# thalesfm/differentiable-renderer

Measured on AMD Instinct MI355X. Metric: Mray/s (fwd+bwd), Cornell 512x512 @64spp depth 8, higher is better.
Workload: dtype f32; 1 GPU; config 3: Cornell 512x512, 64 spp, depth 8, fwd + radiative backprop w.r.t. the albedos; scene 'cornell' (cornell box of render.cpp:26-59) 512x512, 64 spp per GPU, depth 8 (-b 8 -p 1), fwd + radiative-backprop gradients of 4 parameters; program=builtin, parallelism=1 GPU, gpu_max_hw_queues=4 (set by this script before the HIP runtime started)

## Files before the change

differentiable-renderer_amd/csrc/drt_ctx.h:

```cpp
#pragma once

namespace {

struct DevBuf {
    void* p = nullptr;
    size_t cap = 0;
};

struct TimedLaunch {
    int kernel;
    hipEvent_t e0, e1;
};

struct NormalEqRequest {
    const float* d_target = nullptr;
    const float* d_residual = nullptr;
    float* d_jacobian = nullptr;
    double *d_A = nullptr, *d_b = nullptr, *d_loss = nullptr;
    bool cross = false;
    double* d_bias = nullptr;
    float* d_variance = nullptr;
};
struct ParamSetsRequest {
    int n_sets = 0, width = 0;
// ... 33 lines not shown
    float* out_gimg = nullptr;
    drt_hip_stats* stats = nullptr;
    int gimg_param = -1;
    bool tangent = false;
    bool second_image() const { return gimg_param >= 0 || tangent; }
    bool backward = false, dev_out = false, timing = false, want_segments = false, sync = true;
    bool zero_copy = false;
    bool direct_out = false, direct_gimg = false;
    uint64_t done_seq = 0;
    bool copy_kernel = false;
    int n_shards = 1, shard = 0, band = 1;
    uint32_t n_local_pixels = 0;
    size_t n_count_words = 0;
    float* d_out = nullptr;
    float* d_gimg = nullptr;
    size_t off_grad = 0, off_img = 0, off_gimg = 0, off_adj = 0, img_bytes = 0, grad_bytes = 0;
    drt_hip_stats st;
    std::chrono::steady_clock::time_point t0;
};

}

struct drt_hip_ctx {
    int device = 0;
    int n_cu = 256;
    uint64_t device_mem = (uint64_t)288 << 30;
    int mesh_blocks_per_cu = 4;
    hipStream_t stream = nullptr;
    std::string err;

    bool has_scene = false;
    bool has_specular = false;
    bool emissive_bxdf = false;
    int max_colour_param = -1;
    unsigned colour_mask = 0, emission_mask = 0;
    bool prog_ok = false;
    bool prog_sorted = false;
    unsigned long long prog_sig[4] = {0, 0, 0, 0};
    std::string arch = "gfx950";
    int jit_mode = 1;
    uint64_t scene_work = 0;
    std::map<std::string, hipFunction_t> jit_fn;
    std::vector<hipModule_t> jit_modules;
    std::string user_header;
    std::string jit_error;
    double jit_ms = 0;
    int n_params = 0, n_shapes = 0;
    int n_user_params = 0;
    int n_grad_slots = 0;
    std::vector<uint8_t> requires_grad;
    std::vector<drt_material_desc> materials;
    DevScene<float>* d_scene_f = nullptr;
    DevScene<double>* d_scene_d = nullptr;
    float* d_params_f = nullptr;
    double* d_params_d = nullptr;
    bool has_mesh = false;
    DevBvh<float> bvh_f{};
    DevBvh<double> bvh_d{};
    std::vector<void*> mesh_allocs;

    hipStream_t path_stream[2] = {nullptr, nullptr};
    hipEvent_t ev_begin[2] = {nullptr, nullptr}, ev_path[2] = {nullptr, nullptr};
    hipEvent_t ev_lane_free[2] = {nullptr, nullptr};
    bool lane_used[2] = {false, false};
    hipEvent_t ev_params = nullptr;
    bool params_pending[2] = {false, false};
// ... 114 lines not shown
```

differentiable-renderer_amd/csrc/drt_path.h:

```cpp
#pragma once

#include "drt_kernels.h"

#define DRT_DRAW_TABLE (3 * DRT_MAX_DEPTH + 8)

struct PathArgs {
    int32_t W, H, spp;
    int32_t shard, n_shards, band;
    uint32_t Pb, p0, Sb, s0, spr, n_ranges, n_groups;
    int32_t min_bounces, depth_cap, cap_is_roulette, cap_draws;
    uint32_t rr_threshold, seed, rng_stream;
    uint32_t regen_min;
    uint32_t shade_min, descend_min;
    int32_t gimg_param;
    uint32_t gen_rows, gen_clog2;
    uint32_t hist_lds, hist_stride;
    uint32_t gimg_row, pad_gen;
    unsigned long long hist_ovf;
    double p_rr, inv_p_rr;
    double eye[3], fwd[3], right[3], up[3];
    double tan_half, aspect, inv_W, inv_H;
    float p_rr_f, inv_p_rr_f;
    float eye_f[3], fwd_f[3], right_f[3], up_f[3], cs_step_f, ct_step_f;
    __host__ __device__ uint32_t dirs_out() const { return gen_rows; }
// ... 4 lines not shown
{
    uint32_t ly = lp / (uint32_t)a.W, x = lp - ly * (uint32_t)a.W;
    uint32_t y = ly;
    if (a.n_shards > 1) {
        uint32_t b = ly / (uint32_t)a.band, r = ly - b * (uint32_t)a.band;
        y = (b * (uint32_t)a.n_shards + (uint32_t)a.shard) * (uint32_t)a.band + r;
    }
    return y * (uint32_t)a.W + x;
}

template <typename SG>
__device__ inline HitRec<float> path_closest_hit(const DevScene<float>* __restrict__ sc, const ProgRecs<SG::n>& recs, float4 ra, float2 rb)
{
    return closest_hit_prog<SG>(sc, recs, mk<float>(ra.x, ra.y, ra.z), mk<float>(ra.w, rb.x, rb.y));
}
template <typename SG>
__device__ inline HitRec<double> path_closest_hit(const DevScene<double>* __restrict__ sc, const ProgRecs<SG::n, double>& recs, double4 ra, double2 rb)
{
    if (SG::n > 0)
        return closest_hit_sig<SG, double>(recs, mk<double>(ra.x, ra.y, ra.z), mk<double>(ra.w, rb.x, rb.y));
    const double4 ra1[1] = {ra};
    const double2 rb1[1] = {rb};
    HitRec<double> h1[1];
    closest_hit_n<double, 1>(sc, sc->n_shapes, ra1, rb1, h1);
    return h1[0];
}

#define DRT_SIG_CORNELL                                                                                                   \
    ((unsigned long long)DRT_PK_SPHERE | (unsigned long long)DRT_PK_SPHERE << 3 | (unsigned long long)DRT_PK_AX << 6 |    \
     (unsigned long long)DRT_PK_PLANE << 9 | (unsigned long long)DRT_PK_AZ << 12 | (unsigned long long)DRT_PK_AZ << 15 |  \
     (unsigned long long)DRT_PK_AY << 18 | (unsigned long long)DRT_PK_AY << 21 | (unsigned long long)DRT_PK_SPHERE << 24)
#define DRT_NSIG_CORNELL 9
typedef KindSig<DRT_SIG_CORNELL, 0ull, 0ull, 0ull, DRT_NSIG_CORNELL> SigCornell;


template <typename R>
struct PathSceneLds {
    struct {
        int n_shapes, n_materials, n_emitters, n_params;
        DevShape<R> shapes[DRT_MAX_SHAPES];
        DevMaterial<R> materials[DRT_MAX_MATERIALS];
        int emitter_param[DRT_MAX_EMITTERS];
        int flat[DRT_MAX_SHAPES];
    } sc;
    R params[DRT_PATH_LDS_PARAMS * 3];
#ifdef DRT_USER_SHAPES
    R user_q[DRT_MAX_SHAPES][4];
#endif
};

template <typename R, bool ALL_LDS = false>
__device__ inline V3<R> load_param(const PathSceneLds<R>& lds, const R* __restrict__ params, int id)
{
    if (ALL_LDS || id < DRT_PATH_LDS_PARAMS)
        return mk<R>(lds.params[id * 3], lds.params[id * 3 + 1], lds.params[id * 3 + 2]);
    return mk<R>(params[id * 3], params[id * 3 + 1], params[id * 3 + 2]);
}
template <typename R>
struct SetParams {
    const R* p;
};
template <typename R, bool ALL_LDS = false>
__device__ inline V3<R> load_param(const SetParams<R>& set, const R* __restrict__, int id)
{
    return mk<R>(set.p[id * 3], set.p[id * 3 + 1], set.p[id * 3 + 2]);
}
// ... 107 lines not shown
#ifndef DRT_LEAN_PATH_MIN_BLOCKS
#define DRT_LEAN_PATH_MIN_BLOCKS 8
#endif
#ifndef DRT_REGEN_MIN_BLOCKS
#define DRT_REGEN_MIN_BLOCKS 5
#endif
#ifndef DRT_F64_MIN_BLOCKS
#define DRT_F64_MIN_BLOCKS 4
#endif
#ifndef DRT_TANGENT_MIN_BLOCKS
#define DRT_TANGENT_MIN_BLOCKS 6
#endif
#ifndef DRT_TANGENT_REGEN_MIN_BLOCKS
#define DRT_TANGENT_REGEN_MIN_BLOCKS 5
#endif
#ifndef DRT_TANGENT_F64_MIN_BLOCKS
#define DRT_TANGENT_F64_MIN_BLOCKS 3
#endif
#ifndef DRT_TANGENTS2_MIN_BLOCKS
#define DRT_TANGENTS2_MIN_BLOCKS 5
#endif
#ifndef DRT_TANGENTS4_MIN_BLOCKS
#define DRT_TANGENTS4_MIN_BLOCKS 3
#endif
#ifndef DRT_TANGENTS8_MIN_BLOCKS
#define DRT_TANGENTS8_MIN_BLOCKS 2
#endif
#ifndef DRT_GEN_TABLE
#define DRT_GEN_TABLE 408
#endif
template <bool B, typename X, typename Y> struct PickT { typedef X T; };
template <typename X, typename Y> struct PickT<false, X, Y> { typedef Y T; };
struct NoLds { int unused; };
template <typename R> struct GenAcc { typedef double T; };
#ifdef DRT_GEN_F32
template <> struct GenAcc<float> { typedef float T; };
#endif

template <typename R>
struct GenLds {
    R colnz[DRT_PATH_LDS_PARAMS][4];
    R invc[DRT_PATH_LDS_PARAMS][4];
    static __device__ inline const GenLds* over_invc(const R* rows) { return reinterpret_cast<const GenLds*>(rows - DRT_PATH_LDS_PARAMS * 4); }
};

template <typename R, typename SL>
__device__ inline void stage_gen(GenLds<R>& gl, const SL& lds, const DevScene<R>* __restrict__ sc)
{
    for (int p = threadIdx.x; p < DRT_PATH_LDS_PARAMS; p += blockDim.x) {
        const bool in = p < lds.sc.n_params;
        uint32_t zinc = 0, zbits = 0;
#pragma unroll
        for (int ch = 0; ch < 3; ++ch) {
            const R c = in ? lds.params[p * 3 + ch] : R(1);
            const bool zero = zero_channel(c);
            gl.colnz[p][ch] = zero ? R(1) : c;
            gl.invc[p][ch] = zero ? R(0) : R(1) / c;
            zinc |= zero ? 1u << (8 * ch) : 0u;
            zbits |= zero ? 1u << ch : 0u;
        }
        const uint32_t slot = in ? (uint32_t)sc->grad_slot[p] : DRT_SLOT_NONE;
        gl.colnz[p][3] = pid_pack(R(0), zinc);
        gl.invc[p][3] = pid_pack(R(0), slot | zbits << 16);
    }
    __syncthreads();
}
// ... 552 lines not shown
                    a0 = ap;
                if (is_colour) {
                    const uint32_t n = (tg.cnt[p >> 2] >> (8 * (p & 3))) & 0xFFu;
                    const R nf = (R)(int)n;
                    V3<R> dT = mk<R>(Tr.x * (nf * tl.invc[p][0]), Tr.y * (nf * tl.invc[p][1]), Tr.z * (nf * tl.invc[p][2]));
                    const uint32_t zb = __builtin_amdgcn_readfirstlane(tl.inc[p][3]);
                    if (zb) {
                        const bool one = n == 1u;
                        if (zb & 1u) dT.x = (one && (tg.zc & 0xFFu) == 0x1u) ? T.x : R(0);
                        if (zb & 2u) dT.y = (one && (tg.zc & 0xFF00u) == 0x100u) ? T.y : R(0);
                        if (zb & 4u) dT.z = (one && (tg.zc & 0xFF0000u) == 0x10000u) ? T.z : R(0);
                    }
                    tg.acc_set(p, mk<R>(fma_r(dT.x, gE.x, a0.x), fma_r(dT.y, gE.y, a0.y), fma_r(dT.z, gE.z, a0.z)));
                } else
                    tg.acc_set(p, a0);
            }
        }
    }
}

template <typename R>
struct CameraLane {
    R cs0, ct0;
};

template <typename R>
struct PathVertex {
    V3<R> P, nrm, d;
    uint32_t ids;
    int material;
    bool hit, scattered;
};

template <typename R, bool SPEC, int NP, int NC, typename SG, bool FREEZE_BY_ROW = false, bool FIXED = false, bool NO_LIT_BXDF = false>
__device__ inline void path_bounce(const PathArgs& a, const PathSceneLds<R>& lds, const TangentLds<R>& tl, const DevScene<R>* __restrict__ sc,
                                   const R* __restrict__ params, const ProgRecs<SG::n, R>& recs, uint32_t key,
                                   R pk, R inv_pk, uint32_t n_theta, bool next_rr, bool next_cap, bool live, V3<R> g,
                                   typename Q4<R>::T& ra, typename Q2<R>::T& rb, V3<R>& T, V3<R>& L, Tangents<R, NP, NC>& tg,
                                   bool& alive, bool& capped, bool& on_light, uint32_t& light, PathVertex<R>* vo = nullptr,
                                   bool last = false, const float* __restrict__ seed_px = nullptr, const uint32_t* ih = nullptr)
{
    auto draw = [&](uint32_t n) { return ih ? drt_rng_combine(ih[n], key) : rng_draw(a.rng_stream, key, n); };
    const HitRec<R> h = path_closest_hit<SG>(sc, recs, ra, rb);
    const bool hit = live && h.prim >= 0;
    const int prim = h.prim >= 0 ? h.prim : 0;
    const V3<R> o = mk<R>(ra.x, ra.y, ra.z);
    const V3<R> d = mk<R>(ra.w, rb.x, rb.y);
    const V3<R> P = o + d * h.t;
    const DevShape<R>& sh = lds.sc.shapes[prim];
    const uint32_t ids = (uint32_t)sh.pad;
    const uint32_t cid = ids & 0xFFFFu, eid = ids >> 16;
    const bool has_bxdf = cid != DRT_ID_NONE, emits = hit && eid != DRT_ID_NONE;
    on_light = emits && !has_bxdf;
    light = eid;
    if (last && !vo) {
        if constexpr (!NO_LIT_BXDF) if (wave_any(emits && has_bxdf)) {
            if (emits && has_bxdf) {
                if (NP != 0 && seed_px)
                    g = mk<R>((R)seed_px[0], (R)seed_px[1], (R)seed_px[2]);
                add_emission<R, NP, NC>(lds, tl, params, eid, inv_pk, T, g, L, tg);
            }
        }
        alive = false;
        capped = false;
        if constexpr (!FIXED) if (!a.cap_is_roulette) {
            const bool rr_kills = next_rr && draw(n_theta + 2) < a.rr_threshold;
            capped = hit && has_bxdf && !rr_kills;
        }
        return;
    }
    const V3<R> ctr = mk<R>(sh.p[0], sh.p[1], sh.p[2]);
    const V3<R> nsph = normalize(P - ctr);
    const bool is_plane = sh.type == DRT_SHAPE_PLANE;
    V3<R> nrm = mk<R>(is_plane ? ctr.x : nsph.x, is_plane ? ctr.y : nsph.y, is_plane ? ctr.z : nsph.z);
#ifdef DRT_USER_SHAPES
// ... 549 lines not shown
            counts[(size_t)a.n_groups * a.n_ranges + w] = n_capped;
        }
    }
    if constexpr (GEN || SGRAD)
        gen_finish(s_gen, a, gpart);
    else
    if constexpr (NP > 0 && !JAC) {
        const int wv = threadIdx.x / DRT_WAVE;
        double (*red)[DRT_FAST_PARAMS * 3] = s_red;
        if (REGEN) {
            __syncthreads();
            red = reinterpret_cast<double (*)[DRT_FAST_PARAMS * 3]>(&s_film[0][0]);
        }
#pragma unroll
        for (int r = 0; r < NP * 3; ++r) {
            double v = (double)tg.acc[r * DRT_BLOCK];
#pragma unroll
            for (int o2 = DRT_WAVE / 2; o2 > 0; o2 >>= 1)
                v += __shfl_down(v, o2);
            if (lane == 0)
                red[wv][r] = v;
        }
        __syncthreads();
        if (threadIdx.x < DRT_FAST_PARAMS * 3) {
            double v = 0;
            if ((int)threadIdx.x < NP * 3)
                for (int ww = 0; ww < DRT_BLOCK / DRT_WAVE; ++ww)
                    v += red[ww][threadIdx.x];
            gpart[(size_t)blockIdx.x * (DRT_FAST_PARAMS * 3) + threadIdx.x] = v;
        }
    }
}

template <typename R, int NP, int NCR, typename SG>
__global__ void __launch_bounds__(DRT_BLOCK, (SG::n <= DRT_LEAN_MAX_SHAPES ? DRT_LEAN_PATH_MIN_BLOCKS : DRT_LOCKSTEP_GEN_MIN_BLOCKS))
k_path_lean(PathArgs a, const DevScene<R>* __restrict__ sc, const R* __restrict__ params, const float* __restrict__ adjoint,
            double* __restrict__ gpart, double* __restrict__ fpart, uint32_t* __restrict__ counts,
            unsigned long long* __restrict__ total, double* __restrict__ gimg_part)
{
    static_assert(sizeof(R) == 4 && (NP == 0 || NP == 4), "k_path_lean: f32, four parameters in columns or none");
    static_assert(!DRT_JACOBIAN_OF(NCR), "k_path_lean has no Jacobian form");
    (void)gimg_part;
    if (total && blockIdx.x == 0 && threadIdx.x < 8)
        total[threadIdx.x] = 0;
    typedef typename Q4<R>::T R4;
    typedef typename Q2<R>::T R2;
    constexpr int NC = DRT_NC_OF(NCR), ROLES = DRT_ROLES_OF(NCR);
    __shared__ PathSceneLds<R> lds;
    __shared__ double s_red[DRT_BLOCK / DRT_WAVE][DRT_FAST_PARAMS * 3];
    __shared__ TangentLds<R> s_tl;
    stage_path_scene(lds, sc, params);
    const TangentLds<R>& tl = s_tl;
    if (NC > 0)
        stage_tangents(s_tl, lds);

    const uint32_t lane = threadIdx.x & (DRT_WAVE - 1);
    const uint32_t w = grid_wave();
    const uint32_t range = w / a.n_groups, group = w - range * a.n_groups;
    const uint32_t lp = group * DRT_WAVE + lane;
    const bool have = range < a.n_ranges && lp < a.Pb;
    const uint32_t s_begin = range * a.spr;
    const uint32_t s_end = s_begin + a.spr < a.Sb ? s_begin + a.spr : a.Sb;

    Tangents<R, NP, NC> tg;
    __shared__ R s_acc[NP > 0 ? NP * 3 : 1][DRT_BLOCK];
    tg.acc = &s_acc[0][threadIdx.x];
#pragma unroll
    for (int p = 0; p < NP; ++p)
        tg.acc_set(p, mk<R>(R(0), R(0), R(0)));
    double fx = 0, fy = 0, fz = 0;
    uint32_t n_seg = 0;

    uint32_t gpix = 0, px = 0, py = 0;
    V3<R> g = mk<R>(R(1), R(1), R(1));
// ... 4 lines not shown
        if (NP != 0 && adjoint)
            g = mk<R>((R)adjoint[(size_t)gpix * 3], (R)adjoint[(size_t)gpix * 3 + 1], (R)adjoint[(size_t)gpix * 3 + 2]);
    }
    CameraLane<R> cl;
    cl.cs0 = (R)((2. * (double)px * a.inv_W - 1.) * a.aspect * a.tan_half);
    cl.ct0 = (R)((2. * (double)py * a.inv_H - 1.) * a.tan_half);
    constexpr bool ARGS_F32 = DRT_CAMERA_ARGS_F32 != 0 && SG::n <= DRT_LEAN_MAX_SHAPES;
    ProgRecs<SG::n, R> recs;
    __shared__ typename PickT<(SG::n == 0), ProgLds, NoLds>::T s_prog;
    recs.lds = reinterpret_cast<const ProgLds*>(&s_prog);
    if (SG::n > 0)
        recs.template load<SG>(sc);
    if constexpr (SG::n == 0) {
        const DevScene<float>* scf = reinterpret_cast<const DevScene<float>*>(sc);
        if (threadIdx.x < DRT_PROG_SORTED_MAX) {
            s_prog.rec[threadIdx.x] = *reinterpret_cast<const float4*>(scf->sorted[threadIdx.x]);
            s_prog.shape[threadIdx.x] = scf->sorted_shape[threadIdx.x];
        }
        if (threadIdx.x < 8)
            s_prog.kind_begin[threadIdx.x] = scf->kind_begin[threadIdx.x];
        __syncthreads();
    }

    if (range < a.n_ranges) {
        for (uint32_t sl = s_begin; sl < s_end; ++sl) {
            R4 ra;
            R2 rb;
            const uint32_t key = path_camera<R, ARGS_F32>(a, cl, gpix, px, py, sl, ra, rb);
            bool live = have;
            V3<R> T = mk<R>(R(1), R(1), R(1)), L = mk<R>(R(0), R(0), R(0));
            uint32_t end_ids = DRT_ID_NONE;
            if (NC > 0)
                tg.new_path();
            for (int kk = 0; kk < a.depth_cap; ++kk) {
                const uint32_t n_live = (uint32_t)__popcll(wave_ballot(live));
                if (n_live == 0)
                    break;
                n_seg += n_live;
                const uint32_t n_theta = 2u * (uint32_t)kk + 2u;
                const bool next_cap = (kk + 1) >= a.depth_cap;
                bool alive, capped, on_light;
                uint32_t light;
                path_bounce<R, false, NP, NC, SG, (DRT_FREEZE_BY_ROW != 0 && SG::n <= DRT_LEAN_MAX_SHAPES), true, true>(
                    a, lds, tl, sc, params, recs, key, R(1), R(1), n_theta, false, next_cap, live, g, ra, rb, T, L, tg, alive, capped, on_light, light, nullptr, next_cap);
                end_ids = on_light ? light : end_ids;
                live = alive;
            }
            if (wave_any(end_ids != DRT_ID_NONE)) {
                if (end_ids != DRT_ID_NONE)
                    add_emission<R, NP, NC, false, PathSceneLds<R>, ROLES>(lds, tl, params, end_ids, R(1), T, g, L, tg);
            }
            fx += (double)L.x; fy += (double)L.y; fz += (double)L.z;
        }
        if (fpart && have) {
            double* f = fpart + ((size_t)range * 3) * a.Pb + lp;
            f[0] = fx; f[(size_t)a.Pb] = fy; f[(size_t)a.Pb * 2] = fz;
        }
        if (lane == 0) {
            counts[w] = n_seg;
            counts[(size_t)a.n_groups * a.n_ranges + w] = 0;
        }
    }
    if constexpr (NP > 0) {
        const int wv = threadIdx.x / DRT_WAVE;
#pragma unroll
        for (int r = 0; r < NP * 3; ++r) {
            double v = (double)tg.acc[r * DRT_BLOCK];
#pragma unroll
            for (int o2 = DRT_WAVE / 2; o2 > 0; o2 >>= 1)
                v += __shfl_down(v, o2);
            if (lane == 0)
                s_red[wv][r] = v;
        }
        __syncthreads();
        if (threadIdx.x < DRT_FAST_PARAMS * 3) {
            double v = 0;
// ... 706 lines not shown
```

differentiable-renderer_amd/csrc/drt_prog.h:

```cpp
#pragma once

#include "drt_device.h"

__device__ inline float prog_rcp(float x) { return __builtin_amdgcn_rcpf(x); }
__device__ inline double prog_rcp(double x) { return div_r(1.0, x); }
__device__ inline float prog_sqrt(float x) { return __builtin_amdgcn_sqrtf(x); }
__device__ inline double prog_sqrt(double x) { return sqrt_r(x); }

#ifdef DRT_USER_SHAPES
#include "drt_user_shapes.h"
template <int K, typename R>
__device__ inline bool user_intersect(const R* p, V3<R> o, V3<R> d, R& t)
{
    if (K == 0) return drt_user_intersect_0<R>(p, o, d, t);
    return drt_user_intersect_1<R>(p, o, d, t);
}
template <typename R>
__device__ inline V3<R> user_normal(int kind, const R* p, V3<R> P)
{
    if (kind == 0) return drt_user_normal_0<R>(p, P);
    return drt_user_normal_1<R>(p, P);
}
template <typename R>
__device__ inline void user_bxdf(int kind, const R* p, V3<R> n, V3<R> d, R u1, R u2, V3<R>& wo, R& pdf, R& bs)
// ... 111 lines not shown
};

template <typename SG, typename R>
__device__ inline HitRec<R> closest_hit_sig(const ProgRecs<SG::n, R>& recs, V3<R> o, V3<R> d)
{
    const V3<R> inv_d = mk<R>(prog_rcp(d.x), prog_rcp(d.y), prog_rcp(d.z));
    R tmin = (R)INFINITY;
    int prim = -1;
#pragma unroll
    for (int s = 0; s < SG::n; ++s) {
        const int kind = SG::kind(s);
        const typename Q4<R>::T r = recs.r[s];
        if (kind == DRT_PK_AX) prog_test<DRT_PK_AX, R>(r, s, o, d, inv_d, tmin, prim);
        else if (kind == DRT_PK_AY) prog_test<DRT_PK_AY, R>(r, s, o, d, inv_d, tmin, prim);
        else if (kind == DRT_PK_AZ) prog_test<DRT_PK_AZ, R>(r, s, o, d, inv_d, tmin, prim);
        else if (kind == DRT_PK_PLANE) prog_test<DRT_PK_PLANE, R>(r, s, o, d, inv_d, tmin, prim);
#ifdef DRT_USER_SHAPES
        else if (kind >= DRT_PK_USER0 && kind < DRT_PK_USER0 + DRT_MAX_USER_KINDS) {
            const typename Q4<R>::T q = recs.q[s];
            const R p8[8] = {r.x, r.y, r.z, r.w, q.x, q.y, q.z, q.w};
            R t;
            if (kind == DRT_PK_USER0 ? user_intersect<0, R>(p8, o, d, t) : user_intersect<1, R>(p8, o, d, t))
                prog_accept(t, s, tmin, prim);
        }
#endif
        else prog_test<DRT_PK_SPHERE, R>(r, s, o, d, inv_d, tmin, prim);
    }
    HitRec<R> h;
    h.t = tmin;
    h.prim = prim;
    return h;
}

template <typename SG>
__device__ inline HitRec<float> closest_hit_prog(const DevScene<float>* __restrict__ sc, const ProgRecs<SG::n>& recs,
                                                 V3<float> o, V3<float> d)
{
    (void)sc;
    if (SG::n > 0)
        return closest_hit_sig<SG, float>(recs, o, d);
    const V3<float> inv_d = mk<float>(__builtin_amdgcn_rcpf(d.x), __builtin_amdgcn_rcpf(d.y), __builtin_amdgcn_rcpf(d.z));
    float tmin = INFINITY;
    int prim = -1;
    {
        const ProgLds& pl = *recs.lds;
        bool tie = false;
#define DRT_KIND_LOOP(K)                                                              \
        for (int i = pl.kind_begin[K]; i < pl.kind_begin[K + 1]; ++i) {               \
            const float4 r = pl.rec[i];                                               \
            prog_test_tie<K>(r, pl.shape[i], o, d, inv_d, tmin, prim, tie);           \
        }
        DRT_KIND_LOOP(DRT_PK_AX)
        DRT_KIND_LOOP(DRT_PK_AY)
        DRT_KIND_LOOP(DRT_PK_AZ)
        DRT_KIND_LOOP(DRT_PK_PLANE)
        DRT_KIND_LOOP(DRT_PK_SPHERE)
#undef DRT_KIND_LOOP
        if (__any(tie && prim >= 0)) {
#define DRT_KIND_LOOP(K)                                                              \
            for (int i = pl.kind_begin[K]; i < pl.kind_begin[K + 1]; ++i) {           \
                const float4 r = pl.rec[i];                                           \
                prog_resolve_tie<K>(r, pl.shape[i], o, d, inv_d, tmin, prim);         \
            }
            DRT_KIND_LOOP(DRT_PK_AX)
            DRT_KIND_LOOP(DRT_PK_AY)
            DRT_KIND_LOOP(DRT_PK_AZ)
// ... 12 lines not shown
```

differentiable-renderer_amd/csrc/drt_render_impl.h:

```cpp
#pragma once

namespace {

int timing_begin(drt_hip_ctx* ctx, bool on, int kernel)
{
    if (!on)
        return DRT_OK;
    while (ctx->event_pool.size() < ctx->events_used + 2) {
        hipEvent_t e;
        HIPCHK(ctx, hipEventCreate(&e));
        ctx->event_pool.push_back(e);
    }
    TimedLaunch t;
    t.kernel = kernel;
    t.e0 = ctx->event_pool[ctx->events_used++];
    t.e1 = ctx->event_pool[ctx->events_used++];
    HIPCHK(ctx, hipEventRecord(t.e0, ctx->stream));
    ctx->timed.push_back(t);
    return DRT_OK;
}

int timing_end(drt_hip_ctx* ctx, bool on)
{
    if (!on)
// ... 84 lines not shown
        (S).st->launches[K]++;                                                     \
    } while (0)

template <int V>
using IntC = std::integral_constant<int, V>;
template <typename F>
auto with_bool(bool b, F&& f)
{
    return b ? f(std::true_type()) : f(std::false_type());
}
template <int V, int... Vs, typename F>
auto with_int(int v, F&& f)
{
    if constexpr (sizeof...(Vs) == 0)
        return v == V ? f(IntC<V>()) : decltype(f(IntC<V>()))();
    else
        return v == V ? f(IntC<V>()) : with_int<Vs...>(v, f);
}
inline int np_width(int n_params, int general)
{
    return n_params <= 4 ? 4 : (n_params <= 8 ? 8 : general);
}

enum class PathOp { biased, unbiased, mesh, tangent, jacobian, tangents, param_sets, param_sets_along, param_sets_grad, cross };
enum class PathProg { cornell, sorted, scene };
struct PathForm {
    PathOp op;
    bool f64, spec;
    int np, nc;
    bool regen;
    bool loss;
    int roles;
    bool fixed, no_lit_bxdf;
    PathProg prog;
    bool lean() const { return fixed && no_lit_bxdf; }
};

template <typename R>
struct Shard {
    typedef typename Q4<R>::T R4;
    typedef typename Q2<R>::T R2;
    drt_hip_ctx* ctx;
    const drt_camera_desc* cam;
    const drt_render_params* rp;
    const float* d_adjoint;
    float* d_out_rgb;
    bool backward, timing;
    drt_hip_stats* st;
    uint32_t n_local_pixels;
    int D;
    double* film;
    int gimg_param;
    double* gfilm;
    float* d_out_gimg;
    bool fwd_tangent;
    bool keep_sums;
    const NormalEqRequest* neq = nullptr;
    uint32_t neq_blocks = 0;
    int neq_vw = 1;
    int n_dirs = 0;
    const ParamSetsRequest* sets = nullptr;
    bool cross() const { return neq && neq->cross; }
    int jac_rows() const { return cross() ? n_dirs * 6 + 3 : (neq || sets) ? (n_dirs > 0 ? n_dirs : ctx->n_params) * (sets && sets->along ? 6 : 3) : 3; }
    bool sets_grad() const { return sets && sets->grad; }
    bool pixel_sums() const { return gimg_param >= 0 || fwd_tangent || neq || (sets && !sets->grad); }
    const DevScene<R>* d_scene;
// ... 48 lines not shown
    double *grad, *gpart;
    unsigned long long* totals;
    bool path_finished = false;

    int bounces_from(int k) const
    {
        if (!can_fuse)
            return 1;
        const int left = D - k;
        const int forced = tuning().shade_bounces > 0 ? tuning().shade_bounces : (rp->bounces_per_launch > 8 ? 8 : rp->bounces_per_launch);
        if (forced > 0)
            return forced < left ? forced : left;
        double alive = 1.0;
        int n = 0;
        while (n < left && n < 8) {
            alive *= 0.93 * ((k + n + 1) >= rp->min_bounces && (k + n + 1) < D ? 1.0 - rp->absorb : 1.0);
            ++n;
            if (alive < 0.1)
                break;
        }
        return n;
    }
};

inline std::string path_kernel_name(const drt_hip_ctx* ctx, const PathForm& f)
{
    const std::string sg = drt_jit::sig_type(ctx->prog_sig, ctx->n_shapes);
    const char* type = f.f64 ? "double" : "float";
    const char* sp = f.spec ? "true" : "false";
    char name[400];
    if (f.op == PathOp::unbiased)
        snprintf(name, sizeof name, "k_path_unbiased<%s, %s, %d, %s>", type, sp, f.np, sg.c_str());
    else if (f.lean())
        snprintf(name, sizeof name, "k_path_lean<%s, %d, %d, %s>", type, f.np, DRT_NC_ROLES(f.nc, 0, 0) | f.roles << 8, sg.c_str());
    else
        snprintf(name, sizeof name, "k_path<%s, %s, %d, %d, %s, %s%s>", type, sp, f.np,
                 DRT_NC_ROLES(f.nc, 0, 0) | f.roles << 8 | (f.op == PathOp::jacobian ? DRT_NC_JACOBIAN : 0), sg.c_str(), f.regen ? "true" : "false", f.loss ? ", true" : "");
    return name;
}

template <typename R>
unsigned path_dynamic_lds(const PathForm& f, int n_params, unsigned hist_bytes)
{
    const uint32_t n = (uint32_t)std::min(n_params, DRT_PATH_LDS_PARAMS), K = (uint32_t)f.nc;
    if (f.op == PathOp::tangents || f.op == PathOp::cross) return dirs_table_words(n, K) * (unsigned)sizeof(R);
    if (f.op == PathOp::param_sets) return sets_table_words(n, K) * (unsigned)sizeof(R);
    if (f.op == PathOp::param_sets_along) return sets_along_table_words(n, K) * (unsigned)sizeof(R);
    if (f.op == PathOp::param_sets_grad) return hist_bytes + sets_grad_table_words(n, K) * (unsigned)sizeof(R);
    return f.op == PathOp::unbiased ? 0u : hist_bytes;
}

template <typename R>
const void* library_path_kernel(const PathForm& f)
{
    if (f.loss || f.prog == PathProg::scene)
        return nullptr;
    const auto columns = [&f](auto k) {
        if (f.np == DRT_NP_ANY && f.nc == 0) return k(IntC<DRT_NP_ANY>(), IntC<0>());
        if (f.np == 8 && f.nc == 8) return k(IntC<8>(), IntC<8>());
        if (f.np == 4 && f.nc == 3) return k(IntC<4>(), IntC<3>());
        if (f.np == 4 && f.nc == 4) return k(IntC<4>(), IntC<4>());
        if (f.np == 0 && f.nc == 0) return k(IntC<0>(), IntC<0>());
        return (const void*)nullptr;
    };
    if (f.lean()) {
        if constexpr (sizeof(R) == 4) {
            if (f.np == 4 && f.nc == 3 && f.roles == DRT_ROLES_CORNELL)
                return with_bool(f.prog == PathProg::cornell, [](auto cornell) {
                    return (const void*)k_path_lean<R, 4, DRT_NC_ROLES(3, 0, 0) | DRT_ROLES_CORNELL << 8, std::conditional_t<cornell, SigCornell, SigNone>>; });
            if (f.np == 0 && f.nc == 0 && f.roles == 0)
                return with_bool(f.prog == PathProg::cornell, [](auto cornell) {
                    return (const void*)k_path_lean<R, 0, 0, std::conditional_t<cornell, SigCornell, SigNone>>; });
        }
        return nullptr;
    }
    const auto spec_sig = [&f](auto k) {
        return with_bool(f.spec, [&](auto spec) { return with_bool(f.prog == PathProg::cornell, [&](auto cornell) {
            return k(spec, std::conditional_t<cornell, SigCornell, SigNone>()); }); });
    };
    if (f.op == PathOp::jacobian) {
        if (f.regen || f.roles != 0)
            return nullptr;
        const auto jcols = [&f](auto k) {
            if (f.np == 8 && f.nc == 8) return k(IntC<8>(), IntC<8>());
            if (f.np == 4 && f.nc == 3) return k(IntC<4>(), IntC<3>());
            if (f.np == 4 && f.nc == 4) return k(IntC<4>(), IntC<4>());
            return (const void*)nullptr;
        };
        return jcols([&](auto np, auto nc) {
            return spec_sig([](auto spec, auto sg) {
                return (const void*)k_path<R, decltype(spec)::value, decltype(np)::value, decltype(nc)::value | DRT_NC_JACOBIAN, decltype(sg), false>;
            });
        });
    }
    if (f.roles != 0) {
        if constexpr (sizeof(R) == 4) {
            if (f.op == PathOp::biased && !f.spec && !f.regen && f.np == 4 && f.nc == 3 && f.roles == DRT_ROLES_CORNELL)
                return with_bool(f.prog == PathProg::cornell, [](auto cornell) {
                    return (const void*)k_path<R, false, 4, DRT_NC_ROLES(3, 0, 0) | DRT_ROLES_CORNELL << 8, std::conditional_t<cornell, SigCornell, SigNone>, false>; });
        }
        return nullptr;
    }
    if (const int tag = f.op == PathOp::param_sets ? DRT_NP_SETS : (f.op == PathOp::param_sets_along ? DRT_NP_SETS_ALONG
                        : (f.op == PathOp::param_sets_grad ? DRT_NP_SETS_GRAD : (f.op == PathOp::tangents ? DRT_NP_TANGENT : (f.op == PathOp::cross ? DRT_NP_CROSS : 0)))))
        return f.regen ? nullptr : with_int<DRT_NP_SETS, DRT_NP_SETS_ALONG, DRT_NP_SETS_GRAD, DRT_NP_TANGENT, DRT_NP_CROSS>(tag, [&](auto np) {
// ... 67 lines not shown
    f.op = s.unbiased ? PathOp::unbiased : (s.mesh_path ? PathOp::mesh : (s.fwd_tangent ? PathOp::tangent : (s.neq ? PathOp::jacobian : PathOp::biased)));
    f.f64 = sizeof(R) == 8; f.spec = ctx->has_specular;
    f.np = s.fwd_tangent ? DRT_NP_TANGENT : !tangents ? 0 : (gen ? DRT_NP_ANY : np_width(ctx->n_params, DRT_NP_ANY));
    f.nc = !tangents ? 0 : gen ? (s.gimg_param >= 0 ? 1 : 0)
                             : (f.np == 8 ? 8 : (ctx->max_colour_param < 3 ? 3 : 4));
    if (s.neq && s.n_dirs > 0 && !s.mesh_path) {
        f.op = PathOp::tangents;
        f.np = DRT_NP_TANGENT;
        f.nc = s.n_dirs <= 2 ? 2 : (s.n_dirs <= 4 ? 4 : 8);
        if (s.cross()) {
            f.op = PathOp::cross;
            f.np = DRT_NP_CROSS;
        }
    }
    if (s.sets && !s.mesh_path) {
        f.op = PathOp::param_sets;
        f.np = DRT_NP_SETS;
        f.nc = s.sets->width;
        if (s.sets->along) {
            f.op = PathOp::param_sets_along;
            f.np = DRT_NP_SETS_ALONG;
        }
        if (s.sets->grad) {
            f.op = PathOp::param_sets_grad;
            f.np = DRT_NP_SETS_GRAD;
        }
    }
    f.loss = s.loss_l2;
    f.roles = 0;
    if (tuning().path_roles && tangents && !gen && sizeof(R) == 4 && !f.spec && !f.regen && !f.loss && f.op == PathOp::biased && s.gimg_param < 0 && !s.neq &&
        ctx->colour_mask != 0 && ctx->emission_mask != 0)
        f.roles = (int)(ctx->colour_mask | ctx->emission_mask << 8);
    f.fixed = f.no_lit_bxdf = false;
    if (sizeof(R) == 4 && !f.spec && !f.regen && !f.loss && f.op == PathOp::biased && !s.pixel_sums() &&
        ((f.np == 4 && f.roles != 0) || (f.np == 0 && f.nc == 0)) &&
        rp->absorb >= 1.0 && rp->min_bounces == D && !ctx->emissive_bxdf)
        f.fixed = f.no_lit_bxdf = true;
    if (s.use_path && s.loss_l2) {
        s.use_path = false;
        if ((sizeof(R) == 4 || !ctx->user_header.empty()) && !ctx->emissive_bxdf && ctx->jit_mode >= DRT_SPECIALISE_AUTO) {
            s.loss_kernel = jit_function(ctx, path_kernel_name(ctx, f), ctx->jit_mode > DRT_SPECIALISE_AUTO || !ctx->user_header.empty());
            s.use_path = s.loss_kernel != nullptr;
        }
    }
    s.path_gen = s.use_path && gen;
    const bool builtin = tuning().builtin_program && ctx->jit_mode >= 0 && ctx->n_shapes == DRT_NSIG_CORNELL &&
                         ctx->prog_sig[0] == DRT_SIG_CORNELL && !s.loss_kernel && !s.mesh_path &&
                         ctx->user_header.empty();
    f.prog = builtin ? PathProg::cornell : ((s.loss_kernel || !ctx->user_header.empty()) ? PathProg::scene : PathProg::sorted);
    uint64_t cap_default;
    {
        const uint64_t f = sizeof(R) / 4;
        const uint64_t per_path = f * (112u + 8u * (uint64_t)(D > 0 ? D : 1) + (ctx->has_mesh ? 36u : 0u) + (s.unbiased ? (ctx->has_mesh ? 186u : 110u) : 0u)) + 24u;
        const uint64_t budget = std::min<uint64_t>(ctx->device_mem / 8, (uint64_t)32 << 30);
        cap_default = (uint64_t)1 << 22;
        while (cap_default < ((uint64_t)1 << 28) && 2 * cap_default * per_path <= budget)
            cap_default *= 2;
        if (!s.use_path && rp->batch_paths <= 0 && (uint64_t)ctx->ray_a[0].cap < std::min<uint64_t>(cap_default, s.total_paths) * 16u * f) {
            size_t free_b = 0, total_b = 0;
            if (hipMemGetInfo(&free_b, &total_b) == hipSuccess)
                while (cap_default > ((uint64_t)1 << 22) && cap_default * per_path > (uint64_t)free_b / 2)
                    cap_default /= 2;
        }
    }
    uint64_t cap = rp->batch_paths > 0 ? (uint64_t)rp->batch_paths : cap_default;
    if (s.use_path && rp->batch_paths <= 0)
        cap = s.total_paths;
    if (tuning().batch_paths > 0)
        cap = (uint64_t)tuning().batch_paths;
    if (s.neq || s.sets)
// ... 256 lines not shown
    double* fpart = s.film ? (double*)s.fpart_buf->p : (double*)nullptr;
    double* gpix = s.pixel_sums() ? (double*)ctx->gpix.p : (double*)nullptr;
    unsigned long long* ptotal = s.path_finish ? s.totals : (unsigned long long*)nullptr;
    hipStream_t ks = ctx->stream;
    const bool overlap = s.overlap_ok && s.path_finish;
    const int lane2 = ctx->slot & 1;
    if (overlap) {
        ks = ctx->path_stream[lane2];
        if (d_adjoint) {
            HIPCHK(ctx, hipEventRecord(ctx->ev_begin[lane2], ctx->stream));
            HIPCHK(ctx, hipStreamWaitEvent(ks, ctx->ev_begin[lane2], 0));
        }
        if (ctx->lane_used[lane2] && ctx->ev_lane_free[lane2])
            HIPCHK(ctx, hipStreamWaitEvent(ks, ctx->ev_lane_free[lane2], 0));
        if (ctx->params_pending[lane2] && ctx->ev_params) {
            HIPCHK(ctx, hipStreamWaitEvent(ks, ctx->ev_params, 0));
            ctx->params_pending[lane2] = false;
        }
    }
    PathForm form = s.path;
    hipFunction_t jit = s.loss_kernel;
    ctx->scene_work += (uint64_t)a.n_paths * (uint64_t)(s.D > 0 ? s.D : 1);
    if (form.prog == PathProg::sorted && form.op != PathOp::mesh && ctx->jit_mode > 0 && !form.f64 &&
        (ctx->jit_mode > 1 || ctx->scene_work >= DRT_JIT_AFTER_WORK) && (jit = jit_function(ctx, path_kernel_name(ctx, form), ctx->jit_mode > 1)))
        form.prog = PathProg::scene;
    if (form.prog == PathProg::scene && !jit) {
        jit = jit_function(ctx, path_kernel_name(ctx, form), true);
        if (!jit)
            return fail(ctx, DRT_ERR_UNSUPPORTED, ("render: the scene's caller-defined shape kinds did not compile: " + ctx->jit_error).c_str());
    }
    const void* fn = library_path_kernel<R>(form);
    if (!jit && !fn && form.lean()) {
        form.fixed = form.no_lit_bxdf = false;
        fn = library_path_kernel<R>(form);
    }
    if (!jit && !fn && form.roles != 0) {
        form.roles = 0;
        fn = library_path_kernel<R>(form);
    }
    if (!jit && !fn)
        return fail(ctx, DRT_ERR_UNSUPPORTED, "render: the library carries no path kernel of this form");
    st->path_program = form.prog == PathProg::cornell ? DRT_PROGRAM_BUILTIN : (jit ? DRT_PROGRAM_SPECIALISED : DRT_PROGRAM_SORTED);
    int rc;
    if ((rc = timing_begin(ctx, s.timing, DRT_K_PATH)) != DRT_OK) return rc;
    uint32_t* ovf = s.mesh_path ? (uint32_t*)ctx->mesh_ovf[(s.overlap_ok && lane2) ? 1 : 0].p : (uint32_t*)nullptr;
    uint32_t ovf_stride = (uint32_t)gpath * DRT_BLOCK;
    pa.hist_stride = ovf_stride;
    if (gen && hist_ovf_words > 0) {
        DevBuf& hb = s.mesh_path ? ctx->mesh_ovf[(s.overlap_ok && lane2) ? 1 : 0] : ctx->hist_ovf[(s.overlap_ok && lane2) ? 1 : 0];
        const size_t words = (size_t)hist_ovf_words + (s.mesh_path ? (size_t)(DRT_BVH_STACK - DRT_MESH_LDS_STACK) : 0);
        int rce;
        if ((rce = ensure(ctx, hb, words * ovf_stride * sizeof(uint32_t))) != DRT_OK) return rce;
        if (s.mesh_path) {
            ovf = (uint32_t*)hb.p;
            pa.hist_ovf = (unsigned long long)(uintptr_t)(ovf + (size_t)(DRT_BVH_STACK - DRT_MESH_LDS_STACK) * ovf_stride);
        } else
            pa.hist_ovf = (unsigned long long)(uintptr_t)hb.p;
    }
    pa.gimg_row = DRT_SLOT_NONE;
    if (gen && s.gimg_param >= 0 && s.gimg_param < DRT_PATH_LDS_PARAMS && ctx->requires_grad[(size_t)s.gimg_param]) {
        uint32_t row = 0;
        for (int p2 = 0; p2 < s.gimg_param; ++p2)
            row += ctx->requires_grad[(size_t)p2] ? 1u : 0u;
        pa.gimg_row = row;
    }
    if (sets_grad)
// ... 472 lines not shown
```

differentiable-renderer_amd/csrc/drt_scene.h:

```cpp
#pragma once

namespace {

template <typename R4>
int upload_array(drt_hip_ctx* ctx, const std::vector<R4>& host, const R4** dev)
{
    void* p = nullptr;
    hipError_t e = hipMalloc(&p, host.empty() ? 16 : host.size() * sizeof(R4));
    if (e == hipSuccess && !host.empty())
        e = hipMemcpy(p, host.data(), host.size() * sizeof(R4), hipMemcpyHostToDevice);
    if (e != hipSuccess) {
        ctx->err = std::string("mesh upload: ") + hipGetErrorString(e);
        if (p) (void)hipFree(p);
        return DRT_ERR_HIP;
    }
    ctx->mesh_allocs.push_back(p);
    *dev = (const R4*)p;
    return DRT_OK;
}

inline float link_bits(float, uint32_t v) { float f; memcpy(&f, &v, 4); return f; }
inline double link_bits(double, uint32_t v) { return (double)v; }

template <typename R>
// ... 374 lines not shown
                if (sh.type == DRT_SHAPE_PLANE) {
                    const double nn = sqrt(sh.p[0] * sh.p[0] + sh.p[1] * sh.p[1] + sh.p[2] * sh.p[2]);
                    if (nn > 0)
                        extent = std::max(extent, fabs(sh.p[3]) / nn);
                }
                else if (sh.type == DRT_SHAPE_SPHERE)
                    extent = std::max(extent, sqrt(sh.p[0] * sh.p[0] + sh.p[1] * sh.p[1] + sh.p[2] * sh.p[2]) + fabs(sh.p[3]));
            }
            const double pad = std::max(1e-5 * (diag > 0 ? diag : 1.0), 2e-6 * extent);
            const drt_bvh::Built built = drt_bvh::build(tris, DRT_BVH_LDS_NODES, pad);
            if (built.stack_need > DRT_BVH_STACK || built.nodes.size() >= ((size_t)1 << 24))
                return fail(ctx, DRT_ERR_UNSUPPORTED, "scene: the BVH of this mesh needs a deeper traversal stack than the device kernel has");
            if ((rc = upload_bvh<float>(ctx, built, tris, &ctx->bvh_f)) != DRT_OK) return rc;
            if ((rc = upload_bvh<double>(ctx, built, tris, &ctx->bvh_d)) != DRT_OK) return rc;
            ctx->has_mesh = true;
            ctx->max_colour_param = std::max(ctx->max_colour_param, max_face_param);
            ctx->bvh_bytes = (uint64_t)built.nodes.size() * 64 + (uint64_t)tris.size() * 48;
        }
    }
    ctx->scene_work = 0;
    ctx->n_user_params = s->n_params;
    ctx->n_params = n_dev_params;
    ctx->n_shapes = s->n_shapes;
    ctx->requires_grad.assign((size_t)ctx->n_params, 1);
    if (ctx->n_params > s->n_params)
        ctx->requires_grad[(size_t)s->n_params] = 0;
    if (s->requires_grad)
        for (int i = 0; i < s->n_params; ++i)
            ctx->requires_grad[i] = s->requires_grad[i] ? 1 : 0;
    ctx->emissive_bxdf = false;
    for (int i = 0; i < s->n_shapes; ++i)
        if (s->shapes[i].type != DRT_SHAPE_MESH && s->shapes[i].material >= 0 && s->shapes[i].emitter >= 0)
            ctx->emissive_bxdf = true;
    ctx->has_specular = false;
    auto uses = [&](int m) { if (m >= 0 && s->materials[m].type != DRT_BXDF_DIFFUSE) ctx->has_specular = true; };
    for (int i = 0; i < s->n_shapes; ++i) {
        uses(s->shapes[i].material);
        if (s->shapes[i].type == DRT_SHAPE_MESH && s->meshes[s->shapes[i].mesh].face_material)
            for (int t = 0; t < s->meshes[s->shapes[i].mesh].n_triangles; ++t)
                uses(s->meshes[s->shapes[i].mesh].face_material[t]);
    }
    ctx->has_scene = true;
    return DRT_OK;
}

__global__ void __launch_bounds__(DRT_BLOCK) k_set_params(const double* __restrict__ h_params, int n, float* __restrict__ pf, double* __restrict__ pd)
{
    for (int i = blockIdx.x * DRT_BLOCK + threadIdx.x; i < n; i += gridDim.x * DRT_BLOCK) {
        const double v = h_params[i];
        pf[i] = (float)v;
        pd[i] = v;
    }
}

int update_params_one(drt_hip_ctx* ctx, const double* params)
{
    if (!ctx)
        return DRT_ERR_INVALID;
    if (!ctx->has_scene)
        return fail(ctx, DRT_ERR_NO_SCENE, "update_params before upload_scene");
    if (!params)
        return fail(ctx, DRT_ERR_INVALID, "params is NULL");
    HIPCHK(ctx, hipSetDevice(ctx->device));
    const size_t n = (size_t)ctx->n_user_params * 3;
    if (n == 0)
        return DRT_OK;
// ... 27 lines not shown
```

Before: 213,500 Mray/s.

## Specialise last bounce of lean path kernel to a light-only visibility test

Result: faster. 216,300 Mray/s, median of 6 (+1.3%).

```diff
diff --git a/differentiable-renderer_amd/csrc/drt_ctx.h b/differentiable-renderer_amd/csrc/drt_ctx.h
--- a/differentiable-renderer_amd/csrc/drt_ctx.h
+++ b/differentiable-renderer_amd/csrc/drt_ctx.h
@@ -89,6 +89,7 @@
     bool has_scene = false;
     bool has_specular = false;
     bool emissive_bxdf = false;
+    unsigned long long pure_lights = 0;
     int max_colour_param = -1;
     unsigned colour_mask = 0, emission_mask = 0;
     bool prog_ok = false;
diff --git a/differentiable-renderer_amd/csrc/drt_path.h b/differentiable-renderer_amd/csrc/drt_path.h
--- a/differentiable-renderer_amd/csrc/drt_path.h
+++ b/differentiable-renderer_amd/csrc/drt_path.h
@@ -60,6 +60,17 @@
      (unsigned long long)DRT_PK_AY << 18 | (unsigned long long)DRT_PK_AY << 21 | (unsigned long long)DRT_PK_SPHERE << 24)
 #define DRT_NSIG_CORNELL 9
 typedef KindSig<DRT_SIG_CORNELL, 0ull, 0ull, 0ull, DRT_NSIG_CORNELL> SigCornell;
+#ifndef DRT_LEAN_LIGHTS
+#define DRT_LEAN_LIGHTS 1
+#endif
+#define DRT_LIGHTS_CORNELL (DRT_LEAN_LIGHTS != 0 ? 1ull << 8 : 0ull)
+#ifndef DRT_LEAN_PEEL_LAST
+#ifdef DRT_USER_SHAPES
+#define DRT_LEAN_PEEL_LAST 0
+#else
+#define DRT_LEAN_PEEL_LAST 1
+#endif
+#endif
 
 
 template <typename R>
@@ -233,6 +244,7 @@
 template <bool B, typename X, typename Y> struct PickT { typedef X T; };
 template <typename X, typename Y> struct PickT<false, X, Y> { typedef Y T; };
 struct NoLds { int unused; };
+template <bool B> struct BoolT { static constexpr bool value = B; };
 template <typename R> struct GenAcc { typedef double T; };
 #ifdef DRT_GEN_F32
 template <> struct GenAcc<float> { typedef float T; };
@@ -851,7 +863,8 @@
     bool hit, scattered;
 };
 
-template <typename R, bool SPEC, int NP, int NC, typename SG, bool FREEZE_BY_ROW = false, bool FIXED = false, bool NO_LIT_BXDF = false>
+template <typename R, bool SPEC, int NP, int NC, typename SG, bool FREEZE_BY_ROW = false, bool FIXED = false, bool NO_LIT_BXDF = false,
+          unsigned long long LIGHTS = 0ull>
 __device__ inline void path_bounce(const PathArgs& a, const PathSceneLds<R>& lds, const TangentLds<R>& tl, const DevScene<R>* __restrict__ sc,
                                    const R* __restrict__ params, const ProgRecs<SG::n, R>& recs, uint32_t key,
                                    R pk, R inv_pk, uint32_t n_theta, bool next_rr, bool next_cap, bool live, V3<R> g,
@@ -859,7 +872,17 @@
                                    bool& alive, bool& capped, bool& on_light, uint32_t& light, PathVertex<R>* vo = nullptr,
                                    bool last = false, const float* __restrict__ seed_px = nullptr, const uint32_t* ih = nullptr)
 {
+    static_assert(LIGHTS == 0ull || (sizeof(R) == 4 && SG::n > 0 && FIXED && NO_LIT_BXDF), "LIGHTS: k_path_lean's compiled-in program");
     auto draw = [&](uint32_t n) { return ih ? drt_rng_combine(ih[n], key) : rng_draw(a.rng_stream, key, n); };
+    if constexpr (LIGHTS != 0ull) if (last) {
+        constexpr int l0 = __builtin_ctzll(LIGHTS);
+        const int il = light_end_sig<SG, LIGHTS>(recs, mk<R>(ra.x, ra.y, ra.z), mk<R>(ra.w, rb.x, rb.y));
+        on_light = live && il >= 0;
+        light = (uint32_t)lds.sc.shapes[(LIGHTS & (LIGHTS - 1ull)) == 0ull || il < 0 ? l0 : il].pad >> 16;
+        alive = false;
+        capped = false;
+        return;
+    }
     const HitRec<R> h = path_closest_hit<SG>(sc, recs, ra, rb);
     const bool hit = live && h.prim >= 0;
     const int prim = h.prim >= 0 ? h.prim : 0;
@@ -1475,7 +1498,7 @@
     }
 }
 
-template <typename R, int NP, int NCR, typename SG>
+template <typename R, int NP, int NCR, typename SG, unsigned long long LIGHTS = 0ull>
 __global__ void __launch_bounds__(DRT_BLOCK, (SG::n <= DRT_LEAN_MAX_SHAPES ? DRT_LEAN_PATH_MIN_BLOCKS : DRT_LOCKSTEP_GEN_MIN_BLOCKS))
 k_path_lean(PathArgs a, const DevScene<R>* __restrict__ sc, const R* __restrict__ params, const float* __restrict__ adjoint,
             double* __restrict__ gpart, double* __restrict__ fpart, uint32_t* __restrict__ counts,
@@ -1483,6 +1506,7 @@
 {
     static_assert(sizeof(R) == 4 && (NP == 0 || NP == 4), "k_path_lean: f32, four parameters in columns or none");
     static_assert(!DRT_JACOBIAN_OF(NCR), "k_path_lean has no Jacobian form");
+    static_assert(LIGHTS == 0ull || SG::n > 0, "k_path_lean: the light set belongs to a compiled-in program");
     (void)gimg_part;
     if (total && blockIdx.x == 0 && threadIdx.x < 8)
         total[threadIdx.x] = 0;
@@ -1553,6 +1577,30 @@
             uint32_t end_ids = DRT_ID_NONE;
             if (NC > 0)
                 tg.new_path();
+            if constexpr (SG::n > 0 && DRT_LEAN_PEEL_LAST != 0) {
+                const auto vertex = [&](int kk, auto is_last) {
+                    const uint32_t n_theta = 2u * (uint32_t)kk + 2u;
+                    constexpr bool next_cap = decltype(is_last)::value;
+                    bool alive, capped, on_light;
+                    uint32_t light;
+                    path_bounce<R, false, NP, NC, SG, (DRT_FREEZE_BY_ROW != 0 && SG::n <= DRT_LEAN_MAX_SHAPES), true, true, LIGHTS>(
+                        a, lds, tl, sc, params, recs, key, R(1), R(1), n_theta, false, next_cap, live, g, ra, rb, T, L, tg, alive, capped, on_light, light, nullptr, next_cap);
+                    end_ids = on_light ? light : end_ids;
+                    live = alive;
+                };
+                for (int kk = 0; kk < a.depth_cap - 1; ++kk) {
+                    const uint32_t n_live = (uint32_t)__popcll(wave_ballot(live));
+                    if (n_live == 0)
+                        break;
+                    n_seg += n_live;
+                    vertex(kk, BoolT<false>());
+                }
+                const uint32_t n_live = (uint32_t)__popcll(wave_ballot(live));
+                if (a.depth_cap > 0 && n_live != 0) {
+                    n_seg += n_live;
+                    vertex(a.depth_cap - 1, BoolT<true>());
+                }
+            } else
             for (int kk = 0; kk < a.depth_cap; ++kk) {
                 const uint32_t n_live = (uint32_t)__popcll(wave_ballot(live));
                 if (n_live == 0)
@@ -1562,7 +1610,7 @@
                 const bool next_cap = (kk + 1) >= a.depth_cap;
                 bool alive, capped, on_light;
                 uint32_t light;
-                path_bounce<R, false, NP, NC, SG, (DRT_FREEZE_BY_ROW != 0 && SG::n <= DRT_LEAN_MAX_SHAPES), true, true>(
+                path_bounce<R, false, NP, NC, SG, (DRT_FREEZE_BY_ROW != 0 && SG::n <= DRT_LEAN_MAX_SHAPES), true, true, LIGHTS>(
                     a, lds, tl, sc, params, recs, key, R(1), R(1), n_theta, false, next_cap, live, g, ra, rb, T, L, tg, alive, capped, on_light, light, nullptr, next_cap);
                 end_ids = on_light ? light : end_ids;
                 live = alive;
diff --git a/differentiable-renderer_amd/csrc/drt_prog.h b/differentiable-renderer_amd/csrc/drt_prog.h
--- a/differentiable-renderer_amd/csrc/drt_prog.h
+++ b/differentiable-renderer_amd/csrc/drt_prog.h
@@ -167,6 +167,55 @@
     return h;
 }
 
+template <typename SG, int S>
+__device__ inline bool prog_t_sig(const ProgRecs<SG::n, float>& recs, V3<float> o, V3<float> d, V3<float> inv_d, float& t)
+{
+    constexpr int kind = SG::kind(S);
+    constexpr int known = (kind == DRT_PK_AX || kind == DRT_PK_AY || kind == DRT_PK_AZ || kind == DRT_PK_PLANE) ? kind : DRT_PK_SPHERE;
+    static_assert(!(kind >= DRT_PK_USER0 && kind < DRT_PK_USER0 + DRT_MAX_USER_KINDS), "no light set beside caller-defined kinds (shard_plan)");
+    return prog_t<known, float>(recs.r[S], o, d, inv_d, t);
+}
+template <typename SG, unsigned long long LM, int S = 0>
+__device__ inline void light_end_lights(const ProgRecs<SG::n, float>& recs, V3<float> o, V3<float> d, V3<float> inv_d, float& tl, int& il)
+{
+    if constexpr (S < SG::n) {
+        if constexpr ((LM >> S & 1ull) != 0) {
+            float t;
+            if (prog_t_sig<SG, S>(recs, o, d, inv_d, t))
+                prog_accept(t, S, tl, il);
+        }
+        light_end_lights<SG, LM, S + 1>(recs, o, d, inv_d, tl, il);
+    }
+}
+template <typename SG, unsigned long long LM, int S = 0>
+__device__ inline void light_end_others(const ProgRecs<SG::n, float>& recs, V3<float> o, V3<float> d, V3<float> inv_d, float tl, int il, bool& hidden)
+{
+    if constexpr (S < SG::n) {
+        if constexpr ((LM >> S & 1ull) == 0) {
+            constexpr bool lights_before = (LM & ((1ull << S) - 1ull)) != 0, lights_behind = (LM >> S) != 0;
+            float t;
+            if (prog_t_sig<SG, S>(recs, o, d, inv_d, t)) {
+                if (!lights_before) hidden = hidden || (t > 0.f && t <= tl);
+                else if (!lights_behind) hidden = hidden || (t > 0.f && t < tl);
+                else hidden = hidden || (t > 0.f && (t < tl || (t == tl && S < il)));
+            }
+        }
+        light_end_others<SG, LM, S + 1>(recs, o, d, inv_d, tl, il, hidden);
+    }
+}
+template <typename SG, unsigned long long LM>
+__device__ inline int light_end_sig(const ProgRecs<SG::n, float>& recs, V3<float> o, V3<float> d)
+{
+    static_assert(LM != 0 && SG::n > 0 && SG::n <= 64 && (SG::n == 64 || (LM >> (SG::n & 63)) == 0), "light_end_sig: a light set of the program's own shapes");
+    const V3<float> inv_d = mk<float>(prog_rcp(d.x), prog_rcp(d.y), prog_rcp(d.z));
+    float tl = INFINITY;
+    int il = -1;
+    light_end_lights<SG, LM>(recs, o, d, inv_d, tl, il);
+    bool hidden = false;
+    light_end_others<SG, LM>(recs, o, d, inv_d, tl, il, hidden);
+    return hidden ? -1 : il;
+}
+
 template <typename SG>
 __device__ inline HitRec<float> closest_hit_prog(const DevScene<float>* __restrict__ sc, const ProgRecs<SG::n>& recs,
                                                  V3<float> o, V3<float> d)
diff --git a/differentiable-renderer_amd/csrc/drt_render_impl.h b/differentiable-renderer_amd/csrc/drt_render_impl.h
--- a/differentiable-renderer_amd/csrc/drt_render_impl.h
+++ b/differentiable-renderer_amd/csrc/drt_render_impl.h
@@ -140,6 +140,7 @@
     bool loss;
     int roles;
     bool fixed, no_lit_bxdf;
+    unsigned long long lights;
     PathProg prog;
     bool lean() const { return fixed && no_lit_bxdf; }
 };
@@ -254,7 +255,7 @@
     if (f.op == PathOp::unbiased)
         snprintf(name, sizeof name, "k_path_unbiased<%s, %s, %d, %s>", type, sp, f.np, sg.c_str());
     else if (f.lean())
-        snprintf(name, sizeof name, "k_path_lean<%s, %d, %d, %s>", type, f.np, DRT_NC_ROLES(f.nc, 0, 0) | f.roles << 8, sg.c_str());
+        snprintf(name, sizeof name, "k_path_lean<%s, %d, %d, %s, 0x%llxull>", type, f.np, DRT_NC_ROLES(f.nc, 0, 0) | f.roles << 8, sg.c_str(), f.lights);
     else
         snprintf(name, sizeof name, "k_path<%s, %s, %d, %d, %s, %s%s>", type, sp, f.np,
                  DRT_NC_ROLES(f.nc, 0, 0) | f.roles << 8 | (f.op == PathOp::jacobian ? DRT_NC_JACOBIAN : 0), sg.c_str(), f.regen ? "true" : "false", f.loss ? ", true" : "");
@@ -287,12 +288,14 @@
     };
     if (f.lean()) {
         if constexpr (sizeof(R) == 4) {
+            if (f.prog == PathProg::cornell && f.lights != DRT_LIGHTS_CORNELL)
+                return nullptr;
             if (f.np == 4 && f.nc == 3 && f.roles == DRT_ROLES_CORNELL)
                 return with_bool(f.prog == PathProg::cornell, [](auto cornell) {
-                    return (const void*)k_path_lean<R, 4, DRT_NC_ROLES(3, 0, 0) | DRT_ROLES_CORNELL << 8, std::conditional_t<cornell, SigCornell, SigNone>>; });
+                    return (const void*)k_path_lean<R, 4, DRT_NC_ROLES(3, 0, 0) | DRT_ROLES_CORNELL << 8, std::conditional_t<cornell, SigCornell, SigNone>, (cornell ? DRT_LIGHTS_CORNELL : 0ull)>; });
             if (f.np == 0 && f.nc == 0 && f.roles == 0)
                 return with_bool(f.prog == PathProg::cornell, [](auto cornell) {
-                    return (const void*)k_path_lean<R, 0, 0, std::conditional_t<cornell, SigCornell, SigNone>>; });
+                    return (const void*)k_path_lean<R, 0, 0, std::conditional_t<cornell, SigCornell, SigNone>, (cornell ? DRT_LIGHTS_CORNELL : 0ull)>; });
         }
         return nullptr;
     }
@@ -426,10 +429,13 @@
         ctx->colour_mask != 0 && ctx->emission_mask != 0)
         f.roles = (int)(ctx->colour_mask | ctx->emission_mask << 8);
     f.fixed = f.no_lit_bxdf = false;
+    f.lights = 0;
     if (sizeof(R) == 4 && !f.spec && !f.regen && !f.loss && f.op == PathOp::biased && !s.pixel_sums() &&
         ((f.np == 4 && f.roles != 0) || (f.np == 0 && f.nc == 0)) &&
-        rp->absorb >= 1.0 && rp->min_bounces == D && !ctx->emissive_bxdf)
+        rp->absorb >= 1.0 && rp->min_bounces == D && !ctx->emissive_bxdf) {
         f.fixed = f.no_lit_bxdf = true;
+        f.lights = DRT_LEAN_LIGHTS != 0 && ctx->user_header.empty() ? ctx->pure_lights : 0ull;
+    }
     if (s.use_path && s.loss_l2) {
         s.use_path = false;
         if ((sizeof(R) == 4 || !ctx->user_header.empty()) && !ctx->emissive_bxdf && ctx->jit_mode >= DRT_SPECIALISE_AUTO) {
@@ -752,6 +758,7 @@
     const void* fn = library_path_kernel<R>(form);
     if (!jit && !fn && form.lean()) {
         form.fixed = form.no_lit_bxdf = false;
+        form.lights = 0;
         fn = library_path_kernel<R>(form);
     }
     if (!jit && !fn && form.roles != 0) {
diff --git a/differentiable-renderer_amd/csrc/drt_scene.h b/differentiable-renderer_amd/csrc/drt_scene.h
--- a/differentiable-renderer_amd/csrc/drt_scene.h
+++ b/differentiable-renderer_amd/csrc/drt_scene.h
@@ -430,6 +430,11 @@
     for (int i = 0; i < s->n_shapes; ++i)
         if (s->shapes[i].type != DRT_SHAPE_MESH && s->shapes[i].material >= 0 && s->shapes[i].emitter >= 0)
             ctx->emissive_bxdf = true;
+    ctx->pure_lights = 0;
+    if (!ctx->has_mesh && s->n_shapes <= 64)
+        for (int i = 0; i < s->n_shapes; ++i)
+            if (s->shapes[i].material < 0 && s->shapes[i].emitter >= 0)
+                ctx->pure_lights |= 1ull << i;
     ctx->has_specular = false;
     auto uses = [&](int m) { if (m >= 0 && s->materials[m].type != DRT_BXDF_DIFFUSE) ctx->has_specular = true; };
     for (int i = 0; i < s->n_shapes; ++i) {
```
